# Dingyf717/target-allocation-ppo-transformer

Measured on AMD Instinct MI355X. Metric: env-steps/sec (whole node), full PPO rollout, 4096 envs x 16 UAV x 32 tgt per GPU, higher is better.
Workload: dtype f32 policy (f32 MFMA + fp32-accurate split products on the f16 MFMA) + f64 env

## Files before the change

target-allocation-ppo-transformer_amd/csrc/policy_block.hpp:

```cpp
#pragma once
#include "policy_encoder.hpp"

namespace uavhip {
namespace pol {

template <int head, int nout, int DQ = 4, int XT = (S - 1) * SPW>
__device__ void head_mlp(TID_F Smem& sm, const float* __restrict__ P, const APre<DQ>& pw, float* out) {
    const float* W0 = P + kOffs.o[head + 0];
    const float* b0 = P + kOffs.o[head + 1];
    const float* W2 = P + kOffs.o[head + 2];
    const float* b2 = P + kOffs.o[head + 3];
    const int wv = TIDX() >> 6;
    constexpr int kItems = SPW * nout;
    const int item = TIDX() >> 4, k4 = TIDX() & 15;
    const int p = item / nout, a = (item - p * nout) % nout;
    const f32x4 w2 = *reinterpret_cast<const f32x4*>(W2 + a * HID + 4 * k4);
    const float bb2 = b2[a];
    if (wv < HID / 16) linear1<1, true, DQ>(TID_C pw, W0, D, b0, 16 * wv, sm.h, LDH, XT, sm.z, LDZ, 16 * wv, 0);
    __syncthreads();
    if (item < kItems) {
        const f32x4 z = *reinterpret_cast<const f32x4*>(sm.z + p * LDZ + 4 * k4);
        float acc = (w2.x * z.x + w2.y * z.y) + (w2.z * z.z + w2.w * z.w);
        acc = add_xor2(add_xor1(acc));
        acc += __int_as_float(__builtin_amdgcn_mov_dpp(__float_as_int(acc), 0x141, 0xF, 0xF, true));
        acc += __int_as_float(__builtin_amdgcn_mov_dpp(__float_as_int(acc), 0x140, 0xF, 0xF, true));
        if (k4 == 0) out[item] = acc + bb2;
    }
    __syncthreads();
}

struct CatVals {
    float y0, y1, s, p0, p1, c0, c1, lc0, lc1;
};
__device__ __forceinline__ CatVals categorical(float l0, float l1) {
    CatVals c;
    const float m = fmaxf(l0, l1);
    const float e0 = expf(l0 - m), e1 = expf(l1 - m);
    const float den = e0 + e1;
    c.y0 = e0 / den;
    c.y1 = e1 / den;
    c.s = c.y0 + c.y1;
    c.p0 = c.y0 / c.s;
    c.p1 = c.y1 / c.s;
    const float eps = 1.1920928955078125e-07f;
    c.c0 = fminf(fmaxf(c.p0, eps), 1.f - eps);
    c.c1 = fminf(fmaxf(c.p1, eps), 1.f - eps);
    c.lc0 = logf(c.c0);
    c.lc1 = logf(c.c1);
    return c;
}

__device__ __forceinline__ void store_hidden(TID_F const Smem& sm, float* __restrict__ z, int b0) {
    if (TIDX() < SPW * HID / 4) {
        const int p = TIDX() / (HID / 4), q = TIDX() % (HID / 4);
        *reinterpret_cast<f32x4*>(z + (size_t)(b0 + p) * HID + 4 * q) =
            *reinterpret_cast<const f32x4*>(sm.z + p * LDZ + 4 * q);
    }
}

__device__ __forceinline__ void loss_terms(const float (&o)[5], float l0, float l1, float v, float eps_clip,
                                           float* t, float* verr = nullptr) {
    const CatVals c = categorical(l0, l1);
    const float logp = o[0] > 0.f ? c.lc1 : c.lc0;
    const float ratio = expf(logp - o[1]);
    const float A = o[4];
    const float s1 = ratio * A;
    const float s2 = fminf(fmaxf(ratio, 1.f - eps_clip), 1.f + eps_clip) * A;
    const float R = o[3], ov = o[2];
    const float vc = ov + fminf(fmaxf(v - ov, -eps_clip), eps_clip);
    const bool pad = o[0] < 0.f;
    t[0] = pad ? 0.f : fminf(s1, s2);
    t[1] = pad ? 0.f : (v - R) * (v - R);
    t[2] = pad ? 0.f : (vc - R) * (vc - R);
    t[3] = pad ? 0.f : -(c.lc0 * c.p0 + c.lc1 * c.p1);
    if (verr) *verr = pad ? 0.f : fmaxf(fabsf(v - R), fabsf(vc - R));
}
__device__ __forceinline__ void loss_block_sums(TID_F const float* red, float* fpart, float* vpart, int blk) {
    if (TIDX() < 4) {
        float acc = 0.f;
        for (int i = 0; i < SPW; ++i) acc += red[4 * i + TIDX()];
        fpart[blk * 4 + TIDX()] = acc;
    } else if (TIDX() == 4 && vpart) {
        float m = 0.f;
        for (int i = 0; i < SPW; ++i) m = fmaxf(m, red[4 * SPW + i]);
        vpart[blk] = m;
    }
}
__device__ void loss_partials(TID_F Smem& sm, const TrainIO& io, int b0) {
    float* red = sm.x;
    if (TIDX() < SPW) {
        const int p = TIDX();
        float* o = io.smp + (size_t)(b0 + p) * 8;
        const float l0 = sm.logits[2 * p], l1 = sm.logits[2 * p + 1], v = sm.value[p];
        o[5] = l0;
        o[6] = l1;
        o[7] = v;
        const float eps_clip = hyper_f32(io.hyper, UAVHIP_HP_EPS_CLIP, io.eps_clip);
        const float oi[5] = {o[0], o[1], o[2], o[3], o[4]};
        loss_terms(oi, l0, l1, v, eps_clip, red + 4 * p, red + 4 * SPW + p);
    }
    __syncthreads();
    loss_block_sums(TID_C red, io.fpart, io.vpart, b0 / SPW);
}

template <bool TR, bool RING = false>
__device__ __forceinline__ void gather_windows(TID_F Smem& sm, const float* __restrict__ states, int B, const TrainIO& io,
                                               int b0, bool do_actor, const float* __restrict__ rg) {
    {
        constexpr int kEl = (TOK * LDX + NTHR - 1) / NTHR;
        size_t src[kEl];
#pragma unroll
        for (int u = 0; u < kEl; ++u) {
            const int i = TIDX() + u * NTHR, p = (i / LDX) % SPW;
            src[u] = (size_t)(b0 + p);
            if (TR && i < TOK * LDX) src[u] = (size_t)max(io.idx[b0 + p], 0);
        }
        size_t ssrc = 0;
        [[maybe_unused]] bool pad = false;
        if (TR && TIDX() < SPW) {
            const int r = io.idx[b0 + TIDX()];
            pad = r < 0;
            ssrc = (size_t)max(r, 0);
        }
        float v[kEl];
#pragma unroll
        for (int u = 0; u < kEl; ++u) {
            const int i = TIDX() + u * NTHR;
            const int t = i / LDX, k = i - t * LDX, s = t / SPW, p = t - s * SPW;
            v[u] = (i < TOK * LDX && k < IN && b0 + p < B) ? states[(src[u] * S + s) * IN + k] : 0.f;
        }
        float ld[5];
        if (TR && TIDX() < SPW) {
            ld[0] = pad ? -1.f : (float)(io.act_in[ssrc] != 0);
            ld[1] = io.oldlp_in[ssrc];
            ld[2] = io.oldv_in[ssrc];
            ld[3] = io.ret_in[ssrc];
            ld[4] = io.adv_in[ssrc];
        }
#pragma unroll
        for (int u = 0; u < kEl; ++u) {
            const int i = TIDX() + u * NTHR;
            {
                static_assert(LDX == 16 && NTHR % LDX == 0, "one token row = 16 lanes");
                const unsigned long long nz = __ballot(v[u] != 0.f);
                const float rmax = row16_max(fabsf(v[u]));
                if (i < TOK * LDX && (i % LDX) == 0) {
                    const int t = i / LDX, s = t / SPW, p = t - s * SPW;
                    const bool m = (s < S - 1) && ((nz >> (LANE() & 48)) & 0xFFFFull) == 0;
                    sm.mask[p * S + s] = m;
                    sm.tmax[t] = rmax;
                    if (!RING || (u * NTHR) / LDX >= (S - 1) * SPW)
#pragma unroll
                    for (int ti = 0; ti < 2; ++ti)
                        sm.es[ti][t] = (signed char)range_exp(
                            e_bound_v(range_entry(rg, kRgE + 2 * ti), range_entry(rg, kRgE + 2 * ti + 1), rmax));
                    if (TR && do_actor) {
                        io.mask[(size_t)(b0 + p) * S + s] = m ? 1.f : 0.f;
                        io.tmax[(size_t)(b0 + p) * S + s] = rmax;
                    }
                }
            }
            if (i >= TOK * LDX) continue;
            sm.x[i] = v[u];
            if (TR && do_actor) io.xg[(size_t)trow(i / LDX, b0) * 16 + (i % LDX)] = v[u];
        }
        if (TR && do_actor && TIDX() < SPW) {
            float* o = io.smp + (size_t)(b0 + TIDX()) * 8;
            for (int c = 0; c < 5; ++c) o[c] = ld[c];
        }
    }
}

__device__ __forceinline__ float a0f_load(TID_F const float* m) {
    static_assert(TOK <= 128, "two rows per lane");
    const int l = TIDX();
    return l < 64 ? fmaxf(m[l], l + 64 < TOK ? m[l + 64] : 0.f) : 0.f;
}
__device__ __forceinline__ float a0f_finish(TID_F Smem& sm, float v, const float* e, const float* a0) {
    if (TIDX() < 64) {
        const int l = TIDX();
        v = wave_max(v);
        if (l < 2) {
            const OpSc f = a0_sc_v(e[2 * l], e[2 * l + 1], a0[2 * l], a0[2 * l + 1], v);
            sm.a0f[2 * l] = f.sc;
            sm.a0f[2 * l + 1] = f.inv;
        }
        return v;
    }
    return 0.f;
}
__device__ __forceinline__ float a0f_from_max(TID_F Smem& sm, const float* m, const float* e, const float* a0) {
    return a0f_finish(TID_C sm, a0f_load(TID_C m), e, a0);
}
__device__ __forceinline__ float a0f_from_tmax(TID_F Smem& sm) {
    return a0f_from_max(TID_C sm, sm.tmax, sm.rtab + kRtE, sm.rtab + kRtA0);
}

struct EnvOut {
    int auto_reset;
    float* obs;
    double* rew;
    uint8_t* done;
    double* info;
};

enum { kEnvGrp = 1, kEnvWave = 2, kEnvBoth = 3 };
template <bool TR, bool ROWS, int ENV, bool VONLY = false, bool AONLY = false, int ETAG = 0>
__device__ __forceinline__ void policy_block(TID_F Smem& sm, const float* __restrict__ P, const float* __restrict__ states,
                                             int B, const int8_t* __restrict__ actions_in, uint64_t seed,
                                             uint64_t offset, const uint64_t* __restrict__ offset_dev,
                                             int8_t* __restrict__ action_out, float* __restrict__ logp_out,
                                             float* __restrict__ value_out, float* __restrict__ ent_out,
                                             float* __restrict__ logits_out, const TrainIO& io, const RowIO& rio,
                                             const uavhip_env& env, const EnvOut& eo, int bx,
                                             [[maybe_unused]] int greedy_stride = 0) {
    static_assert(!(TR && ROWS), "the training forward recomputes every row");
    static_assert(!ENV || ROWS, "the fused env step follows the rollout forward");
    static_assert(!VONLY || (ROWS && !ENV && !TR), "value only: the inference ring forward");
    static_assert(!AONLY || (ROWS && ENV && !TR && !VONLY), "actor only: the inference ring forward + env step");
    int blk = bx, role = VONLY ? 2 : AONLY ? 1 : 0;
    if constexpr (TR) {
        if (io.split) {
            role = blk < io.split ? 1 : 2;
            if (role == 2) blk -= io.split;
        }
    }
    const bool do_actor = role != 2, do_critic = role != 1;
    const int b0 = blk * SPW;
    [[maybe_unused]] bool critic_first = false;
    if constexpr (TR) critic_first = role == 0 && io.mix && ((blk >> 3) & 1);
    PTR(0);
    [[maybe_unused]] EmbPre ep_a, ep_c;
    [[maybe_unused]] KvPre<kActorTrunk, 0, TR> pkv_a;
    [[maybe_unused]] KvPre<kCriticTrunk, 0, TR> pkv_c;
    if constexpr (TR) {
        if (do_actor && !critic_first) {
            ep_a = embed_load<kActorTrunk>(TID_C P);
            pkv_a = kv_prefetch<kActorTrunk, 0, TR>(TID_C P);
        } else {
            ep_c = embed_load<kCriticTrunk>(TID_C P);
            pkv_c = kv_prefetch<kCriticTrunk, 0, TR>(TID_C P);
        }
    }
    gather_windows<TR, ROWS>(TID_C sm, states, B, io, b0, do_actor, P + kRangeOff);
    if constexpr (!TR) {
        const int pd = (int)TIDX() - (NTHR - kWave);
        if (!actions_in && pd >= 0 && pd < SPW) {
            const unsigned long long c = offset + (offset_dev ? *offset_dev : 0ull) + (unsigned long long)(b0 + pd);
            const u32x4 r = philox(u32x4{(uint32_t)c, (uint32_t)(c >> 32), 0x5eedu, 0x9e37u}, (uint32_t)seed,
                                   (uint32_t)(seed >> 32));
            sm.u01[pd] = u01f(r.x);
            if constexpr (AONLY) {
                if (greedy_stride > 0 && (b0 + pd) % greedy_stride == 0) sm.u01[pd] = -1.f;
            }
        }
    }
    __syncthreads();
    PTR(1);
    if (!ROWS || !do_actor) {
        const float xm = a0f_from_tmax(TID_C sm);
        if (TR && TIDX() == 0 && io.xmax) io.xmax[blk] = xm;
    }
    if (TR && blk == 0 && TIDX() < kRtN && io.rtab_out) io.rtab_out[TIDX()] = sm.rtab[TIDX()];
    const int wv = TIDX() >> 6;
    const float* headw_a = P + kOffs.o[kActorHead];
    const float* headw_c = P + kOffs.o[kCriticHead];
    [[maybe_unused]] const bool env_grp =
        (ENV & kEnvGrp) && env.N <= envgrp::L && env.M <= envgrp::L && b0 + 2 * wv + 1 < B;
    [[maybe_unused]] envgrp::GRegs gR;
    [[maybe_unused]] envgrp::GPending gq;
    if constexpr (ROWS) {
        if (do_actor) {
            RingPre<kActorTrunk> pw[3];
            RowPre<2> rp;
            rows_prologue<kActorTrunk>(TID_C sm, P, pw, rp, rio, b0, [&] { a0f_from_tmax(TID_C sm); });
            PTR(2);
            __syncthreads();
            encoder_layer_rows<kActorTrunk>(TID_C sm, P, pw, rp, rio, b0);
        }
    }
    constexpr int kHd = TR ? 2 : 4;
    APre<kHd> ph;
    [[maybe_unused]] auto actor = [&] {
        if constexpr (TR && !ROWS) {
            embed_apply<kActorTrunk, TR, kEmbH, split_kv<kActorTrunk, 0, TR>()>(TID_C sm, ep_a, io.e[0],
                                                                                           nullptr, b0);
            PTR(2);
            __syncthreads();
            auto hook = [&] {
                if (wv < 4) ph = prefetch<kHd>(TID_C headw_a, D, 16 * wv, 0);
                if (do_critic && !critic_first) {
                    ep_c = embed_load<kCriticTrunk>(TID_C P);
                    pkv_c = kv_prefetch<kCriticTrunk, 0, TR>(TID_C P);
                }
            };
            encoder_layer<kActorTrunk, 0, true, TR, decltype(hook)>(TID_C sm, P, pkv_a, io.L[0], b0, hook);
            __syncthreads();
            PTR(3);
            head_mlp<kActorHead, 2, kHd>(TID_C sm, P, ph, sm.logits);
            store_hidden(TID_C sm, io.z[0], b0);
        }
    };
    if constexpr (TR) {
        if (do_actor && !critic_first) actor();
    } else if (do_actor) {
        if constexpr (!ROWS) {
            APre<2> pkv = prefetch<2>(TID_C P + kOffs.o[layer_param(kActorTrunk, 0, INW)], D, kv_row(wv, 0), 0);
            embed<kActorTrunk, TR>(TID_C sm, P, io.e[0], nullptr, b0);
            PTR(2);
            __syncthreads();
            encoder_layer<kActorTrunk, 0, true, TR>(TID_C sm, P, pkv, io.L[0], b0);
        }
        if constexpr (AONLY && (ENV & kEnvGrp) && !kExpNoEnv) {
            if (env_grp) {
                const int le = tid_env() & 63;
                envgrp::gload_issue(gR, gq, env, b0 + 2 * (int)(tid_env() >> 6) + (le >> 5), le & 31);
            }
        }
        if (wv < 4) ph = prefetch<kHd>(TID_C headw_a, D, 16 * wv, 0);
        __syncthreads();
        PTR(3);
        head_mlp<kActorHead, 2, kHd>(TID_C sm, P, ph, sm.logits);
    }
    PTR(4);
    if (do_critic) {
        if constexpr (ROWS) {
            RingPre<kCriticTrunk> pw[3];
            RowPre<3> rp;
            rows_prologue<kCriticTrunk>(TID_C sm, P, pw, rp, rio, b0);
            __syncthreads();
            encoder_layer_rows<kCriticTrunk>(TID_C sm, P, pw, rp, rio, b0);
        }
        KvPre<kCriticTrunk, 1, TR> pkv;
        if constexpr (!ROWS) {
            if constexpr (TR) {
                embed_apply<kCriticTrunk, TR, kEmbH, split_kv<kCriticTrunk, 0, TR>()>(TID_C sm, ep_c, io.e[1],
                                                                                                 nullptr, b0);
                __syncthreads();
                auto hook = [&] { pkv = kv_prefetch<kCriticTrunk, 1, TR>(TID_C P); };
                encoder_layer<kCriticTrunk, 0, false, TR, decltype(hook)>(TID_C sm, P, pkv_c, io.L[1], b0, hook);
            } else {
                APre<2> pkv0 = prefetch<2>(TID_C P + kOffs.o[layer_param(kCriticTrunk, 0, INW)], D, kv_row(wv, 0), 0);
                embed<kCriticTrunk, TR>(TID_C sm, P, io.e[1], nullptr, b0);
                __syncthreads();
                encoder_layer<kCriticTrunk, 0, false, TR>(TID_C sm, P, pkv0, io.L[1], b0);
            }
        }
        if constexpr (!TR) pkv = kv_prefetch<kCriticTrunk, 1, TR>(TID_C P);
        __syncthreads();
        if constexpr (TR) {
            auto hook = [&] {
                if (wv < 4) ph = prefetch<kHd>(TID_C headw_c, D, 16 * wv, 0);
            };
            encoder_layer<kCriticTrunk, 1, true, TR, decltype(hook)>(TID_C sm, P, pkv, io.L[2], b0, hook);
        } else {
            encoder_layer<kCriticTrunk, 1, true, TR>(TID_C sm, P, pkv, io.L[2], b0);
        }
        if constexpr ((ENV & kEnvGrp) && !kExpNoEnv) {
            if (env_grp) {
                const int le = tid_env() & 63;
                envgrp::gload_issue(gR, gq, env, b0 + 2 * (int)(tid_env() >> 6) + (le >> 5), le & 31);
            }
        }
        if (!TR && wv < 4) ph = prefetch<kHd>(TID_C headw_c, D, 16 * wv, 0);
        __syncthreads();
        PTR(5);
        head_mlp<kCriticHead, 1, kHd>(TID_C sm, P, ph, sm.value);
        PTR(6);
        if (TR) store_hidden(TID_C sm, io.z[1], b0);
    }
    if constexpr (TR) {
        if (critic_first) {
            ep_a = embed_load<kActorTrunk>(TID_C P);
            pkv_a = kv_prefetch<kActorTrunk, 0, TR>(TID_C P);
            __syncthreads();
            actor();
        }
    }
    if (TR) {
        if (role == 0) {
            loss_partials(TID_C sm, io, b0);
        } else if (TIDX() < SPW) {
            float* o = io.smp + (size_t)(b0 + TIDX()) * 8;
            if (do_actor) {
                o[5] = sm.logits[2 * TIDX()];
                o[6] = sm.logits[2 * TIDX() + 1];
            } else {
                o[7] = sm.value[TIDX()];
            }
        }
        return;
    }
    if constexpr (VONLY) {
        if (TIDX() < SPW && b0 + (int)TIDX() < B) value_out[b0 + TIDX()] = sm.value[TIDX()];
        return;
    }
    if (TIDX() < SPW) {
        const int p = TIDX(), b = b0 + p;
        if (b < B) {
            const float l0 = sm.logits[2 * p], l1 = sm.logits[2 * p + 1];
            const float m = fmaxf(l0, l1);
            const float lse = m + logf(expf(l0 - m) + expf(l1 - m));
            const float lp0 = l0 - lse, lp1 = l1 - lse;
            const float p0 = expf(lp0), p1 = expf(lp1);
            int a;
            if (actions_in) {
                a = actions_in[b] != 0;
            } else {
                const float u = sm.u01[p];
                a = u < p0 ? 0 : 1;
                if constexpr (AONLY) {
                    if (u < 0.f) a = l1 > l0;
                }
            }
            if (action_out) action_out[b] = (int8_t)a;
            if (logp_out) logp_out[b] = a ? lp1 : lp0;
            if (ent_out) ent_out[b] = -(p0 * lp0 + p1 * lp1);
            if (value_out) value_out[b] = sm.value[p];
            if (logits_out) { logits_out[2 * b] = l0; logits_out[2 * b + 1] = l1; }
            if (ENV) sm.mask[p] = a;
        }
    }
    PTR(7);
    if constexpr (ENV && kExpNoEnv) {
        __syncthreads();
        for (int i = TIDX(); i < SPW * envdev::kObs; i += NTHR) {
            const int p = i / envdev::kObs, r = i - p * envdev::kObs, s_ = r / IN, k = r - s_ * IN;
            const int e = b0 + p;
            const float v = sm.x[((s_ < S - 1 ? s_ + 1 : S - 1) * SPW + p) * LDX + k];
            if (e < B) envdev::obs_at(eo.obs, e, false)[r] = k == IN - 1 ? 1.0f : v;
        }
    }
    if constexpr (ENV && !kExpNoEnv) {
        __syncthreads();
        PTR(60);
        using namespace envdev;
        const int lane = tid_env() & 63, wve = tid_env() >> 6, e0 = b0 + 2 * wve;
        if constexpr ((ENV & kEnvGrp) != 0) if (env_grp) {
            const int j = lane & 31, g = lane >> 5, e = e0 + g;
            envgrp::GRegs& R = gR;
            R.tab = nullptr;
            R.win = sm.h + (2 * wve + g) * envgrp::kWin;
            envgrp::gload_finish(R, gq, env, e, j);
            PTR(61);
            envgrp::gstep<false, AONLY, ETAG>(R, env, e, j, sm.mask[2 * wve + g], eo.auto_reset, obs_at(eo.obs, e, obs_f16(env)),
                          (AONLY && !eo.rew) ? nullptr : eo.rew + e,
                          eo.done + e, eo.info ? eo.info + (size_t)e * UAVHIP_INFO_COUNT : nullptr);
            PTR(62);
            envgrp::gstore_delta(R, env, e, j);
            PTR(63);
        }
        if constexpr ((ENV & kEnvWave) != 0) if (!env_grp && e0 < B) {
            const bool two = e0 + 1 < B;
            EnvRegs<1> R0, R1;
            R0.row = R1.row = sm.x + 16 * wve;
            load_regs<1, true>(R0, env, e0, lane);
            if (two) load_regs<1, true>(R1, env, e0 + 1, lane);
#pragma unroll
            for (int k = 0; k < 2; ++k) {
                if (k == 1 && !two) break;
                EnvRegs<1>& R = k ? R1 : R0;
                const int e = e0 + k;
                step_once<1, false, AONLY, ETAG>(R, env, e, lane, sm.mask[2 * wve + k], eo.auto_reset,
                                    obs_at(eo.obs, e, obs_f16(env)), (AONLY && !eo.rew) ? nullptr : eo.rew + e,
                                    eo.done + e,
                                    eo.info ? eo.info + (size_t)e * UAVHIP_INFO_COUNT : nullptr);
                store_regs(R, env, e, lane);
            }
        }
    }
}

template <bool TR, bool ROWS = false, int ENV = 0, bool VONLY = false>
__global__ __launch_bounds__(NTHR) void k_policy_forward(const float* __restrict__ P, const float* __restrict__ states,
                                                         int B, const int8_t* __restrict__ actions_in, uint64_t seed,
// ... 16 lines not shown
```

target-allocation-ppo-transformer_amd/csrc/policy_encoder.hpp:

```cpp
#pragma once
#include "policy_core.hpp"

namespace uavhip {
namespace pol {

struct LnOut {
    float *x, *h, *rs;
    int b0, compact;
    bool nt = true;
};
__device__ __forceinline__ int trow(int tok, int b0) { return (b0 + (tok & (SPW - 1))) * S + tok / SPW; }
__device__ __forceinline__ int orow(int tok, int b0, bool compact) {
    return compact ? b0 + (tok & (SPW - 1)) : trow(tok, b0);
}

struct LnPar {
    f32x4 bb, ww, lb;
};
__device__ __forceinline__ f32x4 ln_bias(TID_F const float* __restrict__ bias) {
    return *reinterpret_cast<const f32x4*>(bias + 16 * (TIDX() >> 6) + 4 * (LANE() >> 4));
}
__device__ __forceinline__ LnPar ln_load(TID_F const f32x4 bb, const float* __restrict__ w, const float* __restrict__ b) {
    const int f0 = 16 * (TIDX() >> 6) + 4 * (LANE() >> 4);
    return LnPar{bb, *reinterpret_cast<const f32x4*>(w + f0), *reinterpret_cast<const f32x4*>(b + f0)};
// ... 468 lines not shown
        else if constexpr (TAIL) po = tail_prefetch<trunk, layer, last, TR>(TID_C P);
        PTR(tb + 1 + 3 * c);
        __syncthreads();
        PTR(tb + 2 + 3 * c);
        if constexpr (TR) store_qkv_chunk(TID_C sm, io.qkv, c, qtok0, b0);
        if constexpr (!in_ctx) {
            attention_chunk<trunk, layer>(TID_C sm, c, S - 1, 1, P);
        } else if constexpr (last) {
            f32x4 o;
            int ti = 0, d0 = 0;
            if (TIDX() < 4 * SPW * 4) attention_task(TID_C sm, TIDX() >> 2, S - 1, o, ti, d0);
            if (c == 0) {
                att0[0] = o;
                ti0 = ti;
                d00 = d0;
            } else if (TIDX() < 4 * SPW * 4) {
                const float asc = att_sc<trunk, layer>(sm, ti & 15).sc;
                attention_out(TID_C sm, 0, ti0, d00, att0[0], asc);
                attention_out(TID_C sm, 1, ti, d0, o, asc);
            }
        } else {
            if (c == 0) {
                attention_full_core(TID_C sm, 0, att0);
            } else {
                f32x4 o[3];
                attention_full_core(TID_C sm, 1, o);
                const float asc = att_sc<trunk, layer>(sm, (int)((TIDX() >> 4) & 15)).sc;
                attention_full_store(TID_C sm, 0, att0, asc);
                attention_full_store(TID_C sm, 1, o, asc);
            }
        }
        __syncthreads();
        PTR(tb + 3 + 3 * c);
    }
    if constexpr (TAIL) layer_tail_fwd<trunk, layer, last, TR, F>(TID_C sm, P, po, io, b0, pre_ln2);
}

template <int trunk, int layer, bool last, bool TR = false, class F = NoHook>
__device__ __forceinline__ void encoder_layer(TID_F Smem& sm, const float* __restrict__ P, KvPre<trunk, layer, TR> pkv,
                              const TrainLayerIO& io = TrainLayerIO{}, int b0 = 0, F pre_ln2 = F{}) {
    if constexpr (split_kv<trunk, layer, TR>()) {
        encoder_layer_split<trunk, layer, last, TR, F>(TID_C sm, P, pkv, io, b0, pre_ln2);
        return;
    } else {
    static_assert(!TR, "the training forward's in_proj GEMMs are split products");
    [[maybe_unused]] constexpr int tb = 8 + 16 * (trunk == 0 ? 0 : 1 + layer);
    PTR(tb);
    const float* Win = P + kOffs.o[layer_param(trunk, layer, INW)];
    const float* bin = P + kOffs.o[layer_param(trunk, layer, INB)];
    const int wv = TIDX() >> 6;
    constexpr int CTQ = last ? 1 : S;
    constexpr int DQ = depth<CTQ>();
    constexpr int qtok0 = last ? (S - 1) * SPW : 0;

    TailPre po;
#pragma unroll
    for (int c = 0; c < 2; ++c) {
        APre<DQ> pq;
        if (wv < 4) pq = prefetch<DQ>(TID_C Win, D, 64 * c + 16 * wv, 0);
        linear1<S, false, 2>(TID_C pkv, Win, D, bin, kv_row(wv, c), sm.h, LDH, 0, sm.big, LDB, (1 + (wv >> 2)) * 64 + 16 * (wv & 3), 0);
        if (wv < 4) linear1<CTQ, false, DQ>(TID_C pq, Win, D, bin, 64 * c + 16 * wv, sm.h, LDH, qtok0, sm.big, LDB, 16 * wv, qtok0);
        if (c == 0) pkv = prefetch<2>(TID_C Win, D, kv_row(wv, 1), 0);
        else po = tail_prefetch<trunk, layer, last, TR>(TID_C P);
        PTR(tb + 1 + 3 * c);
        __syncthreads();
        PTR(tb + 2 + 3 * c);
        if (last) attention_chunk<trunk, layer>(TID_C sm, c, S - 1, 1, P);
        else attention_full<trunk, layer>(TID_C sm, c, P);
        __syncthreads();
        PTR(tb + 3 + 3 * c);
    }
    layer_tail_fwd<trunk, layer, last, TR, F>(TID_C sm, P, po, io, b0, pre_ln2);
    }
}

constexpr int kPposFloats = 2 * S * 3 * D;
constexpr int kRowFloats = 5 * D;
struct RowIO {
    float* rp;
    int B, g;
};
constexpr int kPwD = 4;
template <int trunk> constexpr int row_parts() { return trunk == kActorTrunk ? 2 : 3; }
template <int NP>
struct RowPre {
    f32x4 v[2][2 * NP];
    float pp[2][2];
    f32x4 bias[3];
};

template <int trunk, int NP>
__device__ __forceinline__ void ppos_load(TID_F RowPre<NP>& r, const RowIO& rio) {
    const float* pp = rio.rp + (trunk == kActorTrunk ? 0 : S * 3 * D);
#pragma unroll
    for (int c = 0; c < 2; ++c)
#pragma unroll
        for (int u = 0; u < 2; ++u) {
            const int i = (TIDX() + NTHR * u) % (S * 192);
            const int s = i / 192, rr = i - 192 * s, part = rr >> 6, cc = rr & 63;
            r.pp[c][u] = pp[s * 3 * D + part * D + 64 * c + cc];
        }
}
template <int NP>
__device__ __forceinline__ void ppos_stage(TID_F Smem& sm, const RowPre<NP>& r, int c) {
    float* pl = reinterpret_cast<float*>(sm.red);
#pragma unroll
    for (int u = 0; u < 2; ++u) {
        const int i = TIDX() + NTHR * u;
        if (i < S * 192) pl[i] = r.pp[c][u];
    }
}
template <int NP>
__device__ __forceinline__ void ring_item(TID_F int u, int& part, int& tok) {
    const int t2 = (TIDX() >> 4) + 32 * u;
    part = t2 % NP;
    tok = t2 / NP;
}
template <int trunk, int NP>
__device__ __forceinline__ void ring_load(TID_F RowPre<NP>& r, const Smem& sm, const RowIO& rio, int b0, int c) {
    constexpr int ROFF = trunk == kActorTrunk ? 0 : 2 * D;
    const float* slots = rio.rp + kPposFloats;
    const int q = TIDX() & 15;
    int off[2 * NP];
#pragma unroll
    for (int u = 0; u < 2 * NP; ++u) {
        int part, tok;
        ring_item<NP>(TID_C u, part, tok);
        const int s = tok >> 4, p = tok & 15, b = b0 + p;
        const bool ok = b < rio.B && !sm.mask[p * S + s];
        const int slot = (rio.g + 1 + s) % 5;
        off[u] = ok ? (slot * rio.B + b) * kRowFloats + ROFF + part * D + 64 * c + 4 * q : -1;
    }
    __builtin_amdgcn_sched_barrier(0);
#pragma unroll
    for (int u = 0; u < 2 * NP; ++u) {
        const f32x4 v = *reinterpret_cast<const f32x4*>(slots + (off[u] >= 0 ? off[u] : 4 * q));
        r.v[c][u] = off[u] >= 0 ? v : f32x4{0.f, 0.f, 0.f, 0.f};
    }
}

template <int R, int D, class F>
__device__ __forceinline__ void gemm_rows(TID_F f32x4 (&acc)[R], const APre<D> (&pre)[R], const float* __restrict__ W,
                                          int ldw, const int (&row)[R], const float* X, int ldx, int xtok0,
                                          F&& issued) {
    const int l = LANE(), i16 = l & 15, g = l >> 4;
    const float* xp = X + (xtok0 + i16) * ldx + 4 * g;
    f32x4 a[KB][R], b[KB];
#pragma unroll
    for (int p = 0; p < D; ++p) {
#pragma unroll
        for (int r = 0; r < R; ++r) a[p][r] = pre[r].a[p];
        b[p] = *reinterpret_cast<const f32x4*>(xp + 16 * p);
    }
#pragma unroll
    for (int i = 0; i < KB; ++i) {
        if (i + D < KB) {
#pragma unroll
            for (int r = 0; r < R; ++r)
                a[i + D][r] = *reinterpret_cast<const f32x4*>(frag_ptr(TID_C W, ldw, row[r], 0) + 256 * (i + D));
            b[i + D] = *reinterpret_cast<const f32x4*>(xp + 16 * (i + D));
        }
        if (i == (D < KB ? KB - D - 1 : 0)) issued();
#pragma unroll
        for (int j = 0; j < 4; ++j)
#pragma unroll
            for (int r = 0; r < R; ++r) acc[r] = __builtin_amdgcn_mfma_f32_16x16x4f32(a[i][r][j], b[i][j], acc[r], 0, 0, 0);
        __builtin_amdgcn_sched_barrier(0);
    }
}

template <int R, int D_, class F>
__device__ __forceinline__ void hgemm_rows(TID_F f32x4 (&hi)[R], f32x4 (&lo)[R], const HPre<D_> (&pre)[R],
                                           const float* __restrict__ P, int soff, int K, const int (&row)[R],
                                           const _Float16* X, int xtok0, F&& issued) {
    constexpr int NKB = D / 32;
    const int l = LANE(), i16 = l & 15, g = l >> 4;
    const _Float16* xp = X + (xtok0 + i16) * LDP + 8 * (g ^ ((i16 >> 2) & 1));
    f16x8 a1[NKB][R], a2[NKB][R], b1[NKB], b2[NKB];
#pragma unroll
    for (int p = 0; p < D_; ++p)
#pragma unroll
        for (int r = 0; r < R; ++r) {
            a1[p][r] = pre[r].a1[p];
            a2[p][r] = pre[r].a2[p];
        }
    b1[0] = *reinterpret_cast<const f16x8*>(xp);
    b2[0] = *reinterpret_cast<const f16x8*>(xp + kPlane);
#pragma unroll
    for (int i = 0; i < NKB; ++i) {
        if (i + 1 < NKB) {
            b1[i + 1] = *reinterpret_cast<const f16x8*>(xp + 32 * (i + 1));
            b2[i + 1] = *reinterpret_cast<const f16x8*>(xp + 32 * (i + 1) + kPlane);
        }
        if (i + D_ < NKB) {
#pragma unroll
            for (int r = 0; r < R; ++r) {
                const f16x8* wp = hfrag_ptr(TID_C P, soff, K, row[r], 0) + 128 * (i + D_);
                a1[i + D_][r] = wp[0];
                a2[i + D_][r] = wp[64];
            }
        }
        if (i == (D_ < NKB ? NKB - D_ - 1 : 0)) issued();
#pragma unroll
        for (int r = 0; r < R; ++r) {
            hi[r] = __builtin_amdgcn_mfma_f32_16x16x32_f16(a1[i][r], b1[i], hi[r], 0, 0, 0);
            lo[r] = __builtin_amdgcn_mfma_f32_16x16x32_f16(a1[i][r], b2[i], lo[r], 0, 0, 0);
            lo[r] = __builtin_amdgcn_mfma_f32_16x16x32_f16(a2[i][r], b1[i], lo[r], 0, 0, 0);
        }
        __builtin_amdgcn_sched_barrier(0);
    }
}
template <int trunk>
constexpr bool split_ring() { return split_slot(layer_param(trunk, 0, INW)) >= 0; }
template <int trunk>
using RingPre = std::conditional_t<split_ring<trunk>(), HPre<2>, APre<kPwD>>;

template <int trunk, int NP>
__device__ __forceinline__ void encoder_layer_rows(TID_F Smem& sm, const float* __restrict__ P, const RingPre<trunk> (&pw)[3], RowPre<NP>& rp,
                                   const RowIO& rio, int b0) {
    constexpr bool last = trunk == kActorTrunk;
    constexpr int P0 = 3 - NP, ROFF = trunk == kActorTrunk ? 0 : 2 * D;
    [[maybe_unused]] constexpr int tb = 8 + 16 * (trunk == 0 ? 0 : 1);
    PTR(tb);
    const float* Win = P + kOffs.o[layer_param(trunk, 0, INW)];
    const int l = LANE(), i16 = l & 15, g = l >> 4, wv = TIDX() >> 6;
    const int rows[3] = {16 * wv, D + 16 * wv, 2 * D + 16 * wv};
    f32x4 acc[3] = {};
    auto ring_issue = [&] {
        ring_load<trunk>(TID_C rp, sm, rio, b0, 0);
        if (trunk == kActorTrunk) ring_load<trunk>(TID_C rp, sm, rio, b0, 1);
    };
    if constexpr (split_ring<trunk>()) {
        f32x4 lo[3] = {};
        const float inv = es_factor<trunk, 1>(sm, (S - 1) * SPW + i16);
        hgemm_rows<3, 2>(TID_C acc, lo, pw, P, split_slot(layer_param(trunk, 0, INW)), D, rows,
                         reinterpret_cast<const _Float16*>(sm.ctx), (S - 1) * SPW, ring_issue);
#pragma unroll
        for (int j = 0; j < 3; ++j) acc[j] = (acc[j] + lo[j] * kLoScale) * inv;
    } else {
        gemm_rows<3, kPwD>(TID_C acc, pw, Win, D, rows, sm.ctx, LDH, (S - 1) * SPW, ring_issue);
    }
#pragma unroll
    for (int j = 0; j < 3; ++j) acc[j] += rp.bias[j];
    if (b0 + i16 < rio.B) {
        float* dst = rio.rp + kPposFloats + ((size_t)(rio.g % 5) * rio.B + b0 + i16) * kRowFloats + ROFF + 16 * wv + 4 * g;
#pragma unroll
        for (int j = P0; j < 3; ++j) *reinterpret_cast<f32x4*>(dst + (j - P0) * D) = acc[j];
    }
    if (trunk != kActorTrunk) ring_load<trunk>(TID_C rp, sm, rio, b0, 1);
    PTR(tb + 13);
    const float* pl = reinterpret_cast<const float*>(sm.red);
    const int q = TIDX() & 15;
    TailPre po;
#pragma unroll
    for (int c = 0; c < 2; ++c) {
#pragma unroll
        for (int u = 0; u < 2 * NP; ++u) {
            int part, tok;
            ring_item<NP>(TID_C u, part, tok);
            const int bp = part + P0, s = tok >> 4;
            *reinterpret_cast<f32x4*>(sm.big + tok * LDB + bp * 64 + 4 * q) =
                rp.v[c][u] + *reinterpret_cast<const f32x4*>(pl + s * 192 + bp * 64 + 4 * q);
        }
        if ((wv >> 2) == c) {
#pragma unroll
            for (int j = 0; j < 3; ++j) {
                const int col = 64 * j + 16 * (wv & 3) + 4 * g;
                *reinterpret_cast<f32x4*>(sm.big + ((S - 1) * SPW + i16) * LDB + col) =
                    acc[j] + *reinterpret_cast<const f32x4*>(pl + (S - 1) * 192 + col);
            }
        }
        if (c == 1) po = tail_prefetch<trunk, 0, last, false>(TID_C P);
        PTR(tb + 1 + 3 * c);
        __syncthreads();
        PTR(tb + 2 + 3 * c);
        if (c == 0) ppos_stage(TID_C sm, rp, 1);
        if (last) attention_chunk<trunk, 0>(TID_C sm, c, S - 1, 1, P);
        else attention_full<trunk, 0>(TID_C sm, c, P);
        __syncthreads();
        PTR(tb + 3 + 3 * c);
    }
    layer_tail_fwd<trunk, 0, last, false>(TID_C sm, P, po, TrainLayerIO{}, b0);
}

template <int trunk, int NP, class H = NoHook>
__device__ __forceinline__ void rows_prologue(TID_F Smem& sm, const float* __restrict__ P, RingPre<trunk> (&pw)[3],
                                              RowPre<NP>& rp, const RowIO& rio, int b0, H hook = H{}) {
    const int wv = TIDX() >> 6;
    const EmbPre ep = embed_load<trunk>(TID_C P);
    ppos_load<trunk>(TID_C rp, rio);
    const float* Win = P + kOffs.o[layer_param(trunk, 0, INW)];
#pragma unroll
    for (int j = 0; j < 3; ++j) {
        if constexpr (split_ring<trunk>()) pw[j] = hprefetch<2>(TID_C P, split_slot(layer_param(trunk, 0, INW)), D, j * D + 16 * wv, 0);
        else pw[j] = prefetch<kPwD>(TID_C Win, D, j * D + 16 * wv, 0);
    }
    const float* bin = P + kOffs.o[layer_param(trunk, 0, INB)];
#pragma unroll
    for (int j = 0; j < 3; ++j) rp.bias[j] = *reinterpret_cast<const f32x4*>(bin + j * D + 16 * wv + 4 * (LANE() >> 4));
    hook();
    embed_apply<trunk, false, kEmbSplit>(TID_C sm, ep);
    ppos_stage(TID_C sm, rp, 0);
}

}
}
```

target-allocation-ppo-transformer_amd/csrc/rollout_steps.hip:

```cpp
#define UAVHIP_STEPS_TU 1
#define UAVHIP_TID_LAUNDER 1
#include "common.hpp"
#include "env_device.hpp"
#if defined(UAVHIP_POLICY_TRACE) && defined(UAVHIP_ENV_FINE)
namespace uavhip { namespace pol { __device__ unsigned long long g_strace[256 * 2 * 64]; } }
#define UAVHIP_STRACE_DEFINED 1
#define GTR(id)                                                                                  \
    do {                                                                                         \
        if ((tid_x() & 255) == 0 && blockIdx.x < 256)                                        \
            ::uavhip::pol::g_strace[(blockIdx.x * 2 + (tid_x() >> 8)) * 64 + (id)] = __builtin_amdgcn_s_memtime(); \
    } while (0)
#endif
#include "policy_steps.hpp"

namespace uavhip {
namespace pol {

#define UAVHIP_KARGS(Args)                                       \
    typedef const __attribute__((address_space(4))) Args* kargs; \
    kargs ka = (kargs)__builtin_amdgcn_kernarg_segment_ptr();    \
    int bx = blockIdx.x;                                         \
    unsigned tid = threadIdx.x;                                  \
    asm volatile("" : "+s"(ka), "+s"(bx), "+v"(tid));            \
    tid &= NTHR - 1;                                             \
    const Args& a = *(const Args*)ka

template <auto KGrp, auto KWave, class Args>
int launch_env_path(const Args& args, const char* name, hipStream_t stream) {
    const dim3 grid((args.B + SPW - 1) / SPW), block(NTHR);
    if (args.env.N <= envgrp::L && args.env.M <= envgrp::L && args.B % 2 == 0)
        hipLaunchKernelGGL(KGrp, grid, block, 0, stream, args);
    else
        hipLaunchKernelGGL(KWave, grid, block, 0, stream, args);
    return check_launch(name);
}

template <int ENVP>
__global__ __launch_bounds__(NTHR) void k_rollout_steps(const StepsArgs args) {
    __shared__ __attribute__((aligned(16))) Smem sm;
    if (threadIdx.x >= NTHR / 2) __builtin_amdgcn_s_setprio(1);
    if (threadIdx.x == 0) g_tid_zero = 0;
    load_rtab(TID_K sm, args.P);
    for (int t = 0; t < args.seq.n; ++t) {
        __syncthreads();
        UAVHIP_KARGS(StepsArgs);
        const size_t o = (size_t)t * a.B;
        const RowIO r{a.rio.rp, a.rio.B, a.rio.g + t};
        const EnvOut e{a.eo.auto_reset, a.eo.obs + t * a.seq.obs_stride, a.eo.rew + o, a.eo.done + o,
                       a.eo.info ? a.eo.info + o * UAVHIP_INFO_COUNT : nullptr};
        policy_block<false, true, ENVP>(tid, sm, a.P, a.states + t * a.seq.obs_stride, a.B, nullptr, a.seed,
                                        a.offset + t * a.seq.off_stride, a.offset_dev, a.action_out + o, a.logp_out + o,
                                        a.value_out + o, nullptr, nullptr, TrainIO{}, r, a.env, e, bx);
    }
}
#ifdef UAVHIP_POLICY_TRACE
extern "C" int uavhip_steps_trace(unsigned long long* out, int n) {
    return copy_trace(g_ptrace, 256 * 2 * kTraceSlots, out, n);
}
#endif
int launch_rollout_steps(const StepsArgs& sa, hipStream_t stream) {
    return launch_env_path<k_rollout_steps<kEnvGrp>, k_rollout_steps<kEnvWave>>(sa, "k_rollout_steps", stream);
}

__device__ __forceinline__ void post_step(unsigned tid, Smem& sm, int t, double* s_ret, int* s_cnt, int* s_fin,
                                          int* s_all) {
    typedef const __attribute__((address_space(4))) DecodeArgs* kargs;
    kargs ka = (kargs)__builtin_amdgcn_kernarg_segment_ptr();
    int bx = blockIdx.x;
    asm volatile("" : "+s"(ka), "+s"(bx));
    const DecodeArgs& a = *(const DecodeArgs*)ka;
    if (tid < SPW) {
        const int p = tid, e = bx * SPW + p;
        bool fin = true;
        if (e < a.B) {
            const bool was = s_fin[p] != 0;
            if (!was) {
                s_cnt[p] += 1;
                if (a.ep_return) s_ret[p] = s_ret[p] + a.ep_return[e];
            }
            if (a.actions) a.actions[(size_t)t * a.B + e] = was ? (int8_t)-1 : (int8_t)sm.mask[p];
            fin = was || a.finished[e] != 0;
            s_fin[p] = fin;
        }
        const unsigned m = (unsigned)ballot(fin) & 0xffffu;
        if (p == 0) *s_all = m == 0xffffu;
    }
}
template <int ENVP>
__global__ __launch_bounds__(NTHR) void k_decode_steps(const DecodeArgs args) {
    __shared__ __attribute__((aligned(16))) Smem sm;
    __shared__ double s_ret[SPW];
    __shared__ int s_cnt[SPW], s_fin[SPW], s_all;
    if (threadIdx.x >= NTHR / 2) __builtin_amdgcn_s_setprio(1);
    if (threadIdx.x == 0) g_tid_zero = 0;
    load_rtab(TID_K sm, args.P);
    if (threadIdx.x < SPW) {
        const int p = threadIdx.x, e = blockIdx.x * SPW + p;
        const bool fin = e >= args.B || args.env.istate[(long long)e * UAVHIP_IST_COUNT + UAVHIP_IST_UAV_IDX] >= args.env.N;
        s_fin[p] = fin;
        s_cnt[p] = 0;
        s_ret[p] = (e < args.B && args.ep_return) ? args.ep_return[e] : 0.0;
        const unsigned m = (unsigned)ballot(fin) & 0xffffu;
        if (p == 0) s_all = m == 0xffffu;
    }
    int t = 0;
    for (;;) {
        __syncthreads();
        UAVHIP_KARGS(DecodeArgs);
        if (__builtin_amdgcn_readfirstlane(s_all) || t >= a.n_max) break;
        const int slot = (a.rio.g + t) & 1;
        const RowIO r{a.rio.rp, a.rio.B, a.rio.g + t};
        const EnvOut eo{UAVHIP_STEP_HOLD, a.obs2 + (slot ^ 1) * a.obs_stride, a.ep_return, a.finished, nullptr};
        policy_block<false, true, ENVP, false, true>(tid, sm, a.P, a.obs2 + slot * a.obs_stride, a.B, nullptr, a.seed,
                                                     a.offset + t * a.off_stride, a.offset_dev, nullptr, nullptr,
                                                     nullptr, nullptr, nullptr, TrainIO{}, r, a.env, eo, bx,
                                                     a.greedy_stride);
        __syncthreads();
        post_step(tid, sm, t, s_ret, s_cnt, s_fin, &s_all);
        ++t;
    }
    UAVHIP_KARGS(DecodeArgs);
    const int e0 = bx * SPW;
    if (tid < SPW && e0 + (int)tid < a.B) {
        const int p = tid, e = e0 + p;
        a.steps[e] += s_cnt[p];
        a.finished[e] = s_fin[p] != 0;
        if (a.ep_return) a.ep_return[e] = s_ret[p];
    }
    if (a.actions) {
        for (int i = tid; i < (a.n_max - t) * SPW; i += NTHR) {
            const int e = e0 + i % SPW;
            if (e < a.B) a.actions[(size_t)(t + i / SPW) * a.B + e] = -1;
        }
    }
}
int launch_decode_steps(const DecodeArgs& da, hipStream_t stream) {
    return launch_env_path<k_decode_steps<kEnvGrp>, k_decode_steps<kEnvWave>>(da, "k_decode_steps", stream);
}

template <int ENVP>
__global__ __launch_bounds__(NTHR) void k_rollout_actor_steps(const StepsArgs args) {
    __shared__ __attribute__((aligned(16))) Smem sm;
    if (threadIdx.x >= NTHR / 2) __builtin_amdgcn_s_setprio(1);
    if (threadIdx.x == 0) g_tid_zero = 0;
    load_rtab(TID_K sm, args.P);
    for (int t = 0; t < args.seq.n; ++t) {
        __syncthreads();
        UAVHIP_KARGS(StepsArgs);
        const size_t o = (size_t)t * a.B;
        const RowIO r{a.rio.rp, a.rio.B, a.rio.g + t};
        const EnvOut e{a.eo.auto_reset, a.eo.obs + t * a.seq.obs_stride, a.eo.rew + o, a.eo.done + o,
                       a.eo.info ? a.eo.info + o * UAVHIP_INFO_COUNT : nullptr};
        policy_block<false, true, ENVP, false, true, 1>(tid, sm, a.P, a.states + t * a.seq.obs_stride, a.B, nullptr,
                                                     a.seed, a.offset + t * a.seq.off_stride, a.offset_dev,
                                                     a.action_out + o, a.logp_out + o, nullptr, nullptr, nullptr,
                                                     TrainIO{}, r, a.env, e, bx, 0);
    }
}
int launch_rollout_actor_steps(const StepsArgs& sa, hipStream_t stream) {
    return launch_env_path<k_rollout_actor_steps<kEnvGrp>, k_rollout_actor_steps<kEnvWave>>(sa, "k_rollout_actor_steps",
                                                                                          stream);
}

constexpr int kStashVec = 2 * SPW * LDH / 4;
static_assert(LDP * 2 == LDH * 4, "a planes row and an fp32 row are the same bytes");
__device__ __forceinline__ void value_front(TID_F Smem& sm, const float* __restrict__ P, const float* __restrict__ states,
                                            int B, const RowIO& rio, int b0, f32x4* __restrict__ st) {
    PTR(0);
    gather_windows<false, true>(TID_C sm, states, B, TrainIO{}, b0, false, P + kRangeOff);
    __syncthreads();
    PTR(1);
    a0f_from_tmax(TID_C sm);
    {
        RingPre<kCriticTrunk> pw[3];
        RowPre<3> rp;
        rows_prologue<kCriticTrunk>(TID_C sm, P, pw, rp, rio, b0);
        PTR(2);
        __syncthreads();
        encoder_layer_rows<kCriticTrunk>(TID_C sm, P, pw, rp, rio, b0);
    }
    const KvPre<kCriticTrunk, 1, false> pkv = kv_prefetch<kCriticTrunk, 1, false>(TID_C P);
    __syncthreads();
    encoder_layer_split<kCriticTrunk, 1, true, false, NoHook, false>(TID_C sm, P, pkv, TrainLayerIO{}, b0, NoHook{});
    PTR(3);
    const f32x4* cx = reinterpret_cast<const f32x4*>(sm.ctx);
    for (int i = TIDX(); i < kStashVec; i += NTHR) {
        const int h = kStashVec / 2;
        st[i] = i < h ? cx[(S - 1) * SPW * LDH / 4 + i] : cx[i - h];
    }
    PTR(4);
}
template <int CT>
__device__ __forceinline__ void value_head_gemm(TID_F Smem& sm, const float* __restrict__ P, const APre<KB>& pw, int tok0) {
    const int row = 16 * ((TIDX() >> 6) & 3);
    linear1<CT, true, KB>(TID_C pw, P + kOffs.o[kCriticHead + 0], D, P + kOffs.o[kCriticHead + 1], row, sm.h, LDH, tok0,
                         sm.big, LDZ, row, tok0);
}
__global__ __launch_bounds__(NTHR) void k_value_steps(const ValueArgs args) {
    __shared__ __attribute__((aligned(16))) Smem sm;
    if (threadIdx.x >= NTHR / 2) __builtin_amdgcn_s_setprio(1);
    if (threadIdx.x == 0) g_tid_zero = 0;
    load_rtab(TID_K sm, args.P);
    const int nt = args.n + (args.last_values ? 1 : 0);
    for (int t0 = 0; t0 < nt; t0 += kVG) {
        for (int w = 0; w < kVG && t0 + w < nt; ++w) {
            __syncthreads();
            UAVHIP_KARGS(ValueArgs);
            const int t = t0 + w;
            const RowIO r{a.rio.rp, a.rio.B, a.rio.g + t};
            value_front(tid, sm, a.P, a.obs + t * a.obs_stride, a.B, r, bx * SPW,
                        reinterpret_cast<f32x4*>(a.stash) + ((size_t)bx * kVG + w) * kStashVec);
        }
        __syncthreads();
        UAVHIP_KARGS(ValueArgs);
        const int gw = min(kVG, nt - t0), b0 = bx * SPW;
        PTR(5);
        f32x4 res[kVG];
        {
            const f32x4* st = reinterpret_cast<const f32x4*>(a.stash) + (size_t)bx * kVG * kStashVec;
            constexpr int h = kStashVec / 2, kAll = kVG * h, kIt = (kAll + NTHR - 1) / NTHR;
            f32x4* cx = reinterpret_cast<f32x4*>(sm.ctx);
            f32x4 v[kIt];
#pragma unroll
            for (int u = 0; u < kIt; ++u) {
                const int i = min((int)tid + u * NTHR, kAll - 1), w = i / h;
                v[u] = st[w * kStashVec + (i - w * h)];
            }
            const int ro = h + (tid & 15) * (LDH / 4) + 4 * (tid >> 6) + ((tid >> 4) & 3);
#pragma unroll
            for (int w = 0; w < kVG; ++w) res[w] = st[w * kStashVec + ro];
            __builtin_amdgcn_sched_barrier(0);
#pragma unroll
            for (int u = 0; u < kIt; ++u) {
                const int i = tid + u * NTHR;
                if (i < kAll) cx[i] = i / h < gw ? v[u] : f32x4{0.f, 0.f, 0.f, 0.f};
            }
        }
        const TailPre po = tail_prefetch<kCriticTrunk, 1, false, false>(tid, a.P);
        PTR(6);
        __syncthreads();
        layer_tail<kCriticTrunk, 1, false, false, NoHook, 0, true>(tid, sm, a.P, po, TrainLayerIO{}, b0, NoHook{}, 0, res);
        const int wv = tid >> 6, k4 = tid & 15;
        const APre<KB> ph = prefetch<KB>(tid, a.P + kOffs.o[kCriticHead + 0], D, 16 * (wv & 3), 0);
        const f32x4 w2 = *reinterpret_cast<const f32x4*>(a.P + kOffs.o[kCriticHead + 2] + 4 * k4);
        const float bb2 = a.P[kOffs.o[kCriticHead + 3]];
        __syncthreads();
        if (wv < 4) value_head_gemm<3>(tid, sm, a.P, ph, 0);
        else value_head_gemm<2>(tid, sm, a.P, ph, 3 * SPW);
        __syncthreads();
#pragma unroll
        for (int r = 0; r < (TOK * 16 + NTHR - 1) / NTHR; ++r) {
            const int tok = (NTHR / 16) * r + (tid >> 4);
            if (tok < TOK) {
                const f32x4 z = *reinterpret_cast<const f32x4*>(sm.big + tok * LDZ + 4 * k4);
                float acc = (w2.x * z.x + w2.y * z.y) + (w2.z * z.z + w2.w * z.w);
                acc = add_xor2(add_xor1(acc));
                acc += __int_as_float(__builtin_amdgcn_mov_dpp(__float_as_int(acc), 0x141, 0xF, 0xF, true));
                acc += __int_as_float(__builtin_amdgcn_mov_dpp(__float_as_int(acc), 0x140, 0xF, 0xF, true));
                const int w = tok / SPW, b = b0 + (tok & (SPW - 1)), t = t0 + w;
                if (k4 == 0 && w < gw && b < a.B) (t < a.n ? a.values + (size_t)t * a.B : a.last_values)[b] = acc + bb2;
            }
        }
        PTR(7);
    }
}
int launch_value_steps(const ValueArgs& va, hipStream_t stream) {
    hipLaunchKernelGGL(k_value_steps, dim3((va.B + SPW - 1) / SPW), dim3(NTHR), 0, stream, va);
    return check_launch("k_value_steps");
}

}
}
```

Before: 89.11 million.

## Prefetch next step's observation gather in value kernel and hoist loop-invariant embed loads

The value kernel now issues the global loads for the next timestep's observation window into registers while finishing the current step's gather from the previously loaded registers. This overlaps gather latency with compute. It also hoists the loop-invariant embedding and position loads out of the per-step loop. The cost is extra register pressure from carrying the prefetched values, plus a redundant prefetch on the last step. The rows prologue is split into separate load and apply pieces so weight loads can be placed after the gather.

```diff
diff --git a/target-allocation-ppo-transformer_amd/csrc/policy_block.hpp b/target-allocation-ppo-transformer_amd/csrc/policy_block.hpp
--- a/target-allocation-ppo-transformer_amd/csrc/policy_block.hpp
+++ b/target-allocation-ppo-transformer_amd/csrc/policy_block.hpp
@@ -171,6 +171,48 @@
     }
 }
 
+constexpr int kGatherEl = (TOK * LDX + NTHR - 1) / NTHR;
+__device__ __forceinline__ bool gather_item(TID_F int u, int B, int b0, int& off) {
+    const int i = TIDX() + u * NTHR;
+    const int t = i / LDX, k = i - t * LDX, s = t / SPW, p = t - s * SPW;
+    const bool ok = i < TOK * LDX && k < IN && b0 + p < B;
+    off = ((min(b0 + p, B - 1)) * S + min(s, S - 1)) * IN + min(k, IN - 1);
+    return ok;
+}
+__device__ __forceinline__ void gather_offsets(TID_F int (&off)[kGatherEl], int B, int b0) {
+#pragma unroll
+    for (int u = 0; u < kGatherEl; ++u) gather_item(TID_C u, B, b0, off[u]);
+}
+__device__ __forceinline__ void gather_issue(float (&v)[kGatherEl], const float* __restrict__ states,
+                                             const int (&off)[kGatherEl]) {
+#pragma unroll
+    for (int u = 0; u < kGatherEl; ++u) v[u] = states[off[u]];
+}
+__device__ __forceinline__ void gather_finish(TID_F Smem& sm, const float (&v)[kGatherEl], int B, int b0) {
+#pragma unroll
+    for (int u = 0; u < kGatherEl; ++u) {
+        const int i = TIDX() + u * NTHR;
+        int off;
+        const float x = gather_item(TID_C u, B, b0, off) ? v[u] : 0.f;
+        static_assert(LDX == 16 && NTHR % LDX == 0, "one token row = 16 lanes");
+        const unsigned long long nz = __ballot(x != 0.f);
+        const float rmax = row16_max(fabsf(x));
+        if (i < TOK * LDX && (i % LDX) == 0) {
+            const int t = i / LDX, s = t / SPW, p = t - s * SPW;
+            const bool m = (s < S - 1) && ((nz >> (LANE() & 48)) & 0xFFFFull) == 0;
+            sm.mask[p * S + s] = m;
+            sm.tmax[t] = rmax;
+            if ((u * NTHR) / LDX >= (S - 1) * SPW)
+#pragma unroll
+                for (int ti = 0; ti < 2; ++ti)
+                    sm.es[ti][t] =
+                        (signed char)range_exp(e_bound_v(sm.rtab[kRtE + 2 * ti], sm.rtab[kRtE + 2 * ti + 1], rmax));
+        }
+        if (i >= TOK * LDX) continue;
+        sm.x[i] = x;
+    }
+}
+
 __device__ __forceinline__ float a0f_load(TID_F const float* m) {
     static_assert(TOK <= 128, "two rows per lane");
     const int l = TIDX();
diff --git a/target-allocation-ppo-transformer_amd/csrc/policy_encoder.hpp b/target-allocation-ppo-transformer_amd/csrc/policy_encoder.hpp
--- a/target-allocation-ppo-transformer_amd/csrc/policy_encoder.hpp
+++ b/target-allocation-ppo-transformer_amd/csrc/policy_encoder.hpp
@@ -794,6 +794,39 @@
     embed_apply<trunk, false, kEmbSplit>(TID_C sm, ep);
     ppos_stage(TID_C sm, rp, 0);
 }
-
-}
-}
+template <int trunk, int NP>
+__device__ __forceinline__ void rows_prologue_load_emb(TID_F const float* __restrict__ P, EmbPre& ep, RowPre<NP>& rp,
+                                                       const RowIO& rio) {
+    const EmbPre r = embed_load<trunk>(TID_C P);
+    ep.a = r.a;
+    ep.bb = r.bb;
+    ppos_load<trunk>(TID_C rp, rio);
+}
+template <int trunk, int NP>
+__device__ __forceinline__ void rows_prologue_load_w(TID_F const float* __restrict__ P, EmbPre& ep, RingPre<trunk> (&pw)[3],
+                                                     RowPre<NP>& rp) {
+    const int wv = TIDX() >> 6;
+    {
+        const float* pos = P + kOffs.o[trunk + POS];
+#pragma unroll
+        for (int ct = 0; ct < S; ++ct)
+            ep.pp[ct] = *reinterpret_cast<const f32x4*>(pos + ct * D + 16 * wv + 4 * (LANE() >> 4));
+    }
+    const float* Win = P + kOffs.o[layer_param(trunk, 0, INW)];
+#pragma unroll
+    for (int j = 0; j < 3; ++j) {
+        if constexpr (split_ring<trunk>()) pw[j] = hprefetch<2>(TID_C P, split_slot(layer_param(trunk, 0, INW)), D, j * D + 16 * wv, 0);
+        else pw[j] = prefetch<kPwD>(TID_C Win, D, j * D + 16 * wv, 0);
+    }
+    const float* bin = P + kOffs.o[layer_param(trunk, 0, INB)];
+#pragma unroll
+    for (int j = 0; j < 3; ++j) rp.bias[j] = *reinterpret_cast<const f32x4*>(bin + j * D + 16 * wv + 4 * (LANE() >> 4));
+}
+template <int trunk, int NP>
+__device__ __forceinline__ void rows_prologue_apply(TID_F Smem& sm, const EmbPre& ep, const RowPre<NP>& rp) {
+    embed_apply<trunk, false, kEmbSplit>(TID_C sm, ep);
+    ppos_stage(TID_C sm, rp, 0);
+}
+
+}
+}
diff --git a/target-allocation-ppo-transformer_amd/csrc/rollout_steps.hip b/target-allocation-ppo-transformer_amd/csrc/rollout_steps.hip
--- a/target-allocation-ppo-transformer_amd/csrc/rollout_steps.hip
+++ b/target-allocation-ppo-transformer_amd/csrc/rollout_steps.hip
@@ -164,17 +164,38 @@
 
 constexpr int kStashVec = 2 * SPW * LDH / 4;
 static_assert(LDP * 2 == LDH * 4, "a planes row and an fp32 row are the same bytes");
-__device__ __forceinline__ void value_front(TID_F Smem& sm, const float* __restrict__ P, const float* __restrict__ states,
-                                            int B, const RowIO& rio, int b0, f32x4* __restrict__ st) {
+struct FrontPre {
+    f32x4 a, bb;
+    float pp[2][2];
+};
+__device__ __forceinline__ void value_front(TID_F Smem& sm, const float* __restrict__ P, const float* __restrict__ next,
+                                            int B, const RowIO& rio, int b0, f32x4* __restrict__ st,
+                                            float (&xv)[kGatherEl], const FrontPre& keep) {
     PTR(0);
-    gather_windows<false, true>(TID_C sm, states, B, TrainIO{}, b0, false, P + kRangeOff);
-    __syncthreads();
-    PTR(1);
-    a0f_from_tmax(TID_C sm);
     {
+        int off[kGatherEl];
+        gather_offsets(TID_C off, B, b0);
+#pragma unroll
+        for (int u = 0; u < kGatherEl; ++u) asm volatile("" : "+v"(off[u]));
         RingPre<kCriticTrunk> pw[3];
         RowPre<3> rp;
-        rows_prologue<kCriticTrunk>(TID_C sm, P, pw, rp, rio, b0);
+        EmbPre ep;
+        ep.a = keep.a;
+        ep.bb = keep.bb;
+#pragma unroll
+        for (int c = 0; c < 2; ++c)
+#pragma unroll
+            for (int u = 0; u < 2; ++u) rp.pp[c][u] = keep.pp[c][u];
+        float nx[kGatherEl];
+        gather_issue(nx, next, off);
+        gather_finish(TID_C sm, xv, B, b0);
+#pragma unroll
+        for (int u = 0; u < kGatherEl; ++u) xv[u] = nx[u];
+        __syncthreads();
+        PTR(1);
+        rows_prologue_load_w<kCriticTrunk>(TID_C P, ep, pw, rp);
+        a0f_from_tmax(TID_C sm);
+        rows_prologue_apply<kCriticTrunk>(TID_C sm, ep, rp);
         PTR(2);
         __syncthreads();
         encoder_layer_rows<kCriticTrunk>(TID_C sm, P, pw, rp, rio, b0);
@@ -202,14 +223,32 @@
     if (threadIdx.x == 0) g_tid_zero = 0;
     load_rtab(TID_K sm, args.P);
     const int nt = args.n + (args.last_values ? 1 : 0);
+    float xv[kGatherEl];
+    {
+        int off[kGatherEl];
+        gather_offsets(TID_K off, args.B, blockIdx.x * SPW);
+        gather_issue(xv, args.obs, off);
+    }
+    FrontPre keep;
+    {
+        EmbPre ep;
+        RowPre<3> rp;
+        rows_prologue_load_emb<kCriticTrunk>(TID_K args.P, ep, rp, args.rio);
+        keep.a = ep.a;
+        keep.bb = ep.bb;
+#pragma unroll
+        for (int c = 0; c < 2; ++c)
+#pragma unroll
+            for (int u = 0; u < 2; ++u) keep.pp[c][u] = rp.pp[c][u];
+    }
     for (int t0 = 0; t0 < nt; t0 += kVG) {
         for (int w = 0; w < kVG && t0 + w < nt; ++w) {
             __syncthreads();
             UAVHIP_KARGS(ValueArgs);
             const int t = t0 + w;
             const RowIO r{a.rio.rp, a.rio.B, a.rio.g + t};
-            value_front(tid, sm, a.P, a.obs + t * a.obs_stride, a.B, r, bx * SPW,
-                        reinterpret_cast<f32x4*>(a.stash) + ((size_t)bx * kVG + w) * kStashVec);
+            value_front(tid, sm, a.P, a.obs + min(t + 1, nt - 1) * a.obs_stride, a.B, r, bx * SPW,
+                        reinterpret_cast<f32x4*>(a.stash) + ((size_t)bx * kVG + w) * kStashVec, xv, keep);
         }
         __syncthreads();
         UAVHIP_KARGS(ValueArgs);
```

Measured after the change: 89.96 million (median of 6 runs). No clear change (+0.9%).
